# AssemblyAI-Community/MinImagen

Hardware: NVIDIA H100
Metric: denoising steps/sec (SR256 U-Net, batch 32 per GPU per step) (higher is better)
Workload: dtype f16 tensor-core operands, f32 accumulate / residual stream

## Files before the change

minimagen_b200/csrc/conv_tc.cu:

```cuda
#include "conv_tc.cuh"

#include <cuda_runtime.h>
#include <mutex>
#include <stdio.h>

#include "kernels.cuh"
#include "launch.cuh"
#include "ptx.cuh"
#include "sat_half.cuh"
#include "wgmma.cuh"

namespace mi {

namespace {

constexpr int kNumThreads = 384;
constexpr uint32_t kABytes = kConvBlockM * kConvBlockK * 2;
constexpr uint32_t kRingBudget = 192 * 1024;
constexpr uint32_t kAuxBytes = 512;
constexpr uint32_t kSmemMax = 227 * 1024;
constexpr int kProducerRegs = 40;
constexpr int kConsumerRegs = 232;
static_assert(128 * kProducerRegs + 256 * kConsumerRegs <= 65536, "register file overcommitted");
constexpr int kTurnBar = 2;
constexpr int kStatBar = 4;
constexpr uint32_t stat_scratch_bytes(int block_n) { return 2 * 4 * (block_n / 16 > 0 ? block_n / 16 : 1) * 2 * 8; }

template <int BLOCK_N>
struct Cfg {
    static constexpr uint32_t kBBytes = BLOCK_N * kConvBlockK * 2;
    static constexpr uint32_t kStageBytes = kABytes + kBBytes;
    static constexpr int kStages = (kRingBudget / kStageBytes) > 8 ? 8 : (kRingBudget / kStageBytes);
    static constexpr uint32_t kSmemBytes = kStages * kStageBytes + 1024  + kAuxBytes;
};

__device__ __forceinline__ float silu(float v) { return __fdividef(v, 1.0f + __expf(-v)); }

template <int BLOCK_N, bool GN>
__global__ void __launch_bounds__(kNumThreads, 1)
conv_wg_kernel(const __grid_constant__ CUtensorMap tmA, const __grid_constant__ CUtensorMap tmA2,
               const __grid_constant__ CUtensorMap tmB, const __grid_constant__ CUtensorMap tmX,
               const __grid_constant__ CUtensorMap tmX2, const __grid_constant__ ConvTcArgs args,
               const __grid_constant__ GnPrologueArgs gn) {
    using C = Cfg<BLOCK_N>;
    constexpr int STAGES = C::kStages;
    static_assert(2 * STAGES * 8 <= 256, "barrier block overlaps the GroupNorm scratch");
    constexpr bool PP = !GN && BLOCK_N <= 128;
    constexpr int HALVES = PP ? 2 : 1;

    extern __shared__ uint8_t smem_raw[];
    uint8_t* smem = reinterpret_cast<uint8_t*>((reinterpret_cast<uintptr_t>(smem_raw) + 1023) & ~uintptr_t(1023));
    uint64_t* bars = reinterpret_cast<uint64_t*>(smem + STAGES * C::kStageBytes);
    uint64_t* full_bar = bars;
    uint64_t* empty_bar = bars + STAGES;

    const int warp = threadIdx.x >> 5;
    const int lane = threadIdx.x & 31;
    const int wg = threadIdx.x >> 7;
    int* err = args.err_flag;

    if (threadIdx.x == 0) {
        ptx::prefetch_tensormap(&tmB);
        if (!GN) {
            ptx::prefetch_tensormap(&tmA);
            ptx::prefetch_tensormap(&tmA2);
        }
        for (int i = 0; i < STAGES; ++i) {
            ptx::mbar_init(&full_bar[i], GN ? 5 : 1);
            ptx::mbar_init(&empty_bar[i], PP ? 1 : 2);
        }
        ptx::fence_barrier_init();
    }
    __syncthreads();
    pdl_wait();

    const int num_tap_kb = args.num_taps * args.chunks_per_tap;
    const int num_kb = num_tap_kb + args.x_chunks;
    const int tiles_m = args.tiles_w * args.tiles_h * args.tiles_b;
    const int total_tiles = tiles_m * args.tiles_n;
    const int BW = 1 << args.bw_log2, BH = 1 << args.bh_log2;
    const int BB = kConvBlockM >> (args.bw_log2 + args.bh_log2);

    if (wg == 0) {
        if constexpr (!GN) {
            ptx::setmaxnreg_dec<kProducerRegs>();
            if (warp == 0) {
                int stage = 0;
                uint32_t phase = 0;
                for (int tile = blockIdx.x; tile < total_tiles; tile += gridDim.x) {
                    const int nt = tile % args.tiles_n;
                    const int mt = tile / args.tiles_n;
                    const int w0 = (mt % args.tiles_w) * BW;
                    const int h0 = ((mt / args.tiles_w) % args.tiles_h) * BH;
                    const int b0 = (mt / (args.tiles_w * args.tiles_h)) * BB;
                    const int n0 = nt * BLOCK_N;
                    for (int kb = 0; kb < num_kb; ++kb) {
                        ptx::mbar_wait(&empty_bar[stage], phase ^ 1, err, 100 + stage);
                        if (ptx::elect_one()) {
                            uint8_t* sa = smem + stage * C::kStageBytes;
                            uint8_t* sb = sa + kABytes;
                            ptx::mbar_arrive_expect_tx(&full_bar[stage], C::kStageBytes);
                            if (kb < num_tap_kb) {
                                const int t = kb / args.chunks_per_tap, j = kb - t * args.chunks_per_tap;
                                const int cw = w0 * args.in_stride + args.dw[t], ch = h0 * args.in_stride + args.dh[t];
                                if (j < args.a_split)
                                    ptx::tma_load_5d(&tmA, &full_bar[stage], sa, args.a_chan_off + j * kConvBlockK, cw, ch,
                                                     args.ph[t], b0);
                                else
                                    ptx::tma_load_5d(&tmA2, &full_bar[stage], sa,
                                                     args.a_chan_off2 + (j - args.a_split) * kConvBlockK, cw, ch, args.ph[t], b0);
                            } else {
                                const int jx = kb - num_tap_kb;
                                if (jx < args.x_split)
                                    ptx::tma_load_5d(&tmX, &full_bar[stage], sa, args.x_chan_off + jx * kConvBlockK, w0, h0, 0, b0);
                                else
                                    ptx::tma_load_5d(&tmX2, &full_bar[stage], sa,
                                                     args.x_chan_off2 + (jx - args.x_split) * kConvBlockK, w0, h0, 0, b0);
                            }
                            ptx::tma_load_2d(&tmB, &full_bar[stage], sb, kb * kConvBlockK, n0);
                        }
                        if (++stage == STAGES) { stage = 0; phase ^= 1; }
                    }
                }
                pdl_trigger();
            }
        } else {
            float* s_mean = reinterpret_cast<float*>(reinterpret_cast<uint8_t*>(bars) + 256);
            float* s_rstd = s_mean + 32;
            float* sA = reinterpret_cast<float*>(reinterpret_cast<uint8_t*>(bars) + kAuxBytes);
            const int tt = threadIdx.x;
            const int lq = tt & 7;
            const int prow = tt >> 3;
            const int C0 = gn.C0, C1 = gn.C1, Ctot = C0 + C1, Cg = Ctot / gn.groups;
            const int H = args.H, W = args.W;
            float* sB = sA + Ctot;
            int stage = 0;
            uint32_t phase = 0;
            int cur_b = -1;
            for (int tile = blockIdx.x; tile < total_tiles; tile += gridDim.x) {
                const int nt = tile % args.tiles_n;
                const int mt = tile / args.tiles_n;
                const int w0 = (mt % args.tiles_w) * BW;
                const int h0 = ((mt / args.tiles_w) % args.tiles_h) * BH;
                const int b = mt / (args.tiles_w * args.tiles_h);
                const int n0 = nt * BLOCK_N;
                if (b != cur_b) {
                    ptx::bar_sync(1, 128);
                    if (tt < gn.groups) {
                        const int g = tt;
                        double su = 0.0, sq = 0.0;
                        const int lo = g * Cg, hi = lo + Cg;
                        const int lo0 = min(lo, C0), hi0 = min(hi, C0);
                        for (int e = lo0 / 16; e < hi0 / 16; ++e) {
                            su += gn.stats0[((long long)b * (C0 / 16) + e) * 2];
                            sq += gn.stats0[((long long)b * (C0 / 16) + e) * 2 + 1];
                        }
                        const int lo1 = max(lo, C0) - C0, hi1 = max(hi, C0) - C0;
                        for (int e = lo1 / 16; e < hi1 / 16; ++e) {
                            su += (double)gn.scale1 * gn.stats1[((long long)b * (C1 / 16) + e) * 2];
                            sq += (double)gn.scale1 * (double)gn.scale1 * gn.stats1[((long long)b * (C1 / 16) + e) * 2 + 1];
                        }
                        const double n = (double)Cg * H * W;
                        const double mean = su / n;
                        double var = sq / n - mean * mean;
                        if (var < 0) var = 0;
                        s_mean[g] = (float)mean;
                        s_rstd[g] = (float)(1.0 / sqrt(var + (double)gn.eps));
                    }
                    ptx::bar_sync(1, 128);
                    for (int cc = tt; cc < Ctot; cc += 128) {
                        const int g = cc / Cg;
                        float a = s_rstd[g] * gn.gamma[cc];
                        float bb = gn.beta[cc] - s_mean[g] * a;
                        if (gn.scale_shift) {
                            const float sc = gn.scale_shift[(long long)b * gn.ss_ld + cc] + 1.0f;
                            const float shv = gn.scale_shift[(long long)b * gn.ss_ld + Ctot + cc];
                            a *= sc;
                            bb = bb * sc + shv;
                        }
                        if (cc >= C0) a *= gn.scale1;
                        sA[cc] = a;
                        sB[cc] = bb;
                    }
                    cur_b = b;
                    ptx::bar_sync(1, 128);
                }
                const long long img = (long long)b * H * W;
                for (int kb = 0; kb < num_kb; ++kb) {
                    const int t = kb / args.chunks_per_tap, j = kb - t * args.chunks_per_tap;
                    const int dh = args.dh[t], dw = args.dw[t];
                    const float* cA = sA + j * kConvBlockK + lq * 8;
                    const float* cB = sB + j * kConvBlockK + lq * 8;
                    const float4 a0 = *reinterpret_cast<const float4*>(cA), a1 = *reinterpret_cast<const float4*>(cA + 4);
                    const float4 b0 = *reinterpret_cast<const float4*>(cB), b1 = *reinterpret_cast<const float4*>(cB + 4);
                    const bool first = j < args.a_split;
                    const int Cs = first ? C0 : C1;
                    const float* src = (first ? gn.src0 + (long long)j * kConvBlockK
                                              : gn.src1 + (long long)(j - args.a_split) * kConvBlockK) + img * Cs + lq * 8;

                    ptx::mbar_wait(&empty_bar[stage], phase ^ 1, err, 600 + stage);
                    uint8_t* sa = smem + stage * C::kStageBytes;
                    if (warp == 0 && ptx::elect_one()) {
                        ptx::mbar_arrive_expect_tx(&full_bar[stage], C::kBBytes);
                        ptx::tma_load_2d(&tmB, &full_bar[stage], sa + kABytes, kb * kConvBlockK, n0);
                    }
                    float4 x0[8], x1[8];
                    bool ok[8];
#pragma unroll
                    for (int i = 0; i < 8; ++i) {
                        const int m = i * 16 + prow;
                        const int gw = w0 + (m & (BW - 1)) + dw;
                        const int gh = h0 + ((m >> args.bw_log2) & (BH - 1)) + dh;
                        ok[i] = gh >= 0 && gh < H && gw >= 0 && gw < W;
                        if (ok[i]) {
                            const float4* s4 = reinterpret_cast<const float4*>(src + ((long long)gh * W + gw) * Cs);
                            x0[i] = __ldg(s4);
                            x1[i] = __ldg(s4 + 1);
                        }
                    }
#pragma unroll
                    for (int i = 0; i < 8; ++i) {
                        const int m = i * 16 + prow;
                        uint4 o = make_uint4(0u, 0u, 0u, 0u);
                        if (ok[i]) {
                            const __half2 h0_ = sat_half2(silu(fmaf(x0[i].x, a0.x, b0.x)), silu(fmaf(x0[i].y, a0.y, b0.y)));
                            const __half2 h1_ = sat_half2(silu(fmaf(x0[i].z, a0.z, b0.z)), silu(fmaf(x0[i].w, a0.w, b0.w)));
                            const __half2 h2_ = sat_half2(silu(fmaf(x1[i].x, a1.x, b1.x)), silu(fmaf(x1[i].y, a1.y, b1.y)));
                            const __half2 h3_ = sat_half2(silu(fmaf(x1[i].z, a1.z, b1.z)), silu(fmaf(x1[i].w, a1.w, b1.w)));
                            o.x = *reinterpret_cast<const uint32_t*>(&h0_); o.y = *reinterpret_cast<const uint32_t*>(&h1_);
                            o.z = *reinterpret_cast<const uint32_t*>(&h2_); o.w = *reinterpret_cast<const uint32_t*>(&h3_);
                        }
                        *reinterpret_cast<uint4*>(sa + m * 128 + ((lq ^ (m & 7)) << 4)) = o;
                    }
                    ptx::fence_proxy_async_smem();
                    __syncwarp();
                    if (lane == 0) ptx::mbar_arrive(&full_bar[stage]);
                    if (++stage == STAGES) { stage = 0; phase ^= 1; }
                }
            }
            pdl_trigger();
        }
    } else {
        if constexpr (!GN) ptx::setmaxnreg_inc<kConsumerRegs>();
        const int cw = wg - 1;
        const int wq = warp & 3;
        const int cq = 2 * (lane & 3);
        float acc[HALVES][BLOCK_N / 2];
        int stage = 0;
        uint32_t phase = 0;
        auto skip = [&](int n) {
            stage += n % STAGES;
            phase ^= (uint32_t)(n / STAGES) & 1u;
            if (stage >= STAGES) { stage -= STAGES; phase ^= 1; }
        };
        if (PP) skip(cw * num_kb);
        int bw_r[2 * HALVES], bh_r[2 * HALVES], bb_r[2 * HALVES], bb_warp[HALVES];
#pragma unroll
        for (int h = 0; h < HALVES; ++h) {
            const int m_warp = (PP ? h : cw) * 64 + wq * 16;
            bb_warp[h] = m_warp >> (args.bw_log2 + args.bh_log2);
#pragma unroll
            for (int r = 0; r < 2; ++r) {
                const int m = m_warp + (lane >> 2) + 8 * r;
                bw_r[2 * h + r] = m & (BW - 1);
                bh_r[2 * h + r] = (m >> args.bw_log2) & (BH - 1);
                bb_r[2 * h + r] = m >> (args.bw_log2 + args.bh_log2);
            }
        }
        constexpr int NQ = BLOCK_N / 16 > 0 ? BLOCK_N / 16 : 1;
        const bool tile_stats = PP && args.stats != nullptr && BB == 1;
        double* st_red = reinterpret_cast<double*>(reinterpret_cast<uint8_t*>(bars) + kAuxBytes);
        const bool vec = args.out_sc == 1 && ((reinterpret_cast<uintptr_t>(args.out_f32) & 7) == 0) &&
                         ((reinterpret_cast<uintptr_t>(args.residual) & 7) == 0) &&
                         ((reinterpret_cast<uintptr_t>(args.out_f16) & 3) == 0);

        for (int tile = blockIdx.x + (PP ? cw : 0) * gridDim.x; tile < total_tiles; tile += (PP ? 2 : 1) * gridDim.x) {
            const int nt = tile % args.tiles_n;
            const int mt = tile / args.tiles_n;
            const int n0 = nt * BLOCK_N;
            if (PP && tile != (int)blockIdx.x) ptx::bar_sync(kTurnBar + cw, 256);
            int prev = -1;
            for (int kb = 0; kb < num_kb; ++kb) {
                ptx::mbar_wait(&full_bar[stage], phase, err, 300 + stage);
                const uint32_t sa = ptx::smem_u32(smem + stage * C::kStageBytes);
                const uint64_t db = ptx::make_sw128_desc(sa + kABytes);
                ptx::wg_fence();
#pragma unroll
                for (int k = 0; k < kConvBlockK / 16; ++k)
#pragma unroll
                    for (int h = 0; h < HALVES; ++h) {
                        const uint64_t da = ptx::make_sw128_desc(sa + (PP ? h : cw) * (64 * 128));
                        ptx::Wgmma<BLOCK_N, 0>::run(acc[h], da + 2 * k, db + 2 * k, (kb | k) != 0);
                    }
                ptx::wg_commit();
                ptx::wg_wait<1>();
                if (prev >= 0 && (threadIdx.x & 127) == 0) ptx::mbar_arrive(&empty_bar[prev]);
                prev = stage;
                if (++stage == STAGES) { stage = 0; phase ^= 1; }
            }
            if (PP && tile + (int)gridDim.x < total_tiles) ptx::bar_arrive(kTurnBar + (cw ^ 1), 256);
            if (PP) skip(num_kb);
            ptx::wg_wait<0>();
#pragma unroll
            for (int h = 0; h < HALVES; ++h) ptx::wg_fence_regs(acc[h]);
            if (prev >= 0 && (threadIdx.x & 127) == 0) ptx::mbar_arrive(&empty_bar[prev]);

            const int tw0 = (mt % args.tiles_w) * BW;
            const int th0 = ((mt / args.tiles_w) % args.tiles_h) * BH;
            const int tb0 = (mt / (args.tiles_w * args.tiles_h)) * BB;
            const bool fast = vec && n0 + BLOCK_N <= args.n_valid;
#pragma unroll
            for (int hf = 0; hf < HALVES; ++hf) {
                bool valid[2];
                long long pix[2];
#pragma unroll
                for (int r = 0; r < 2; ++r) {
                    const int w = tw0 + bw_r[2 * hf + r], h = th0 + bh_r[2 * hf + r], b = tb0 + bb_r[2 * hf + r];
                    valid[r] = (b < args.B) && (h < args.H) && (w < args.W);
                    pix[r] = (long long)b * args.out_sb + (long long)h * args.out_sh + (long long)w * args.out_sw;
                }
                const float* a = acc[hf];
                float st_s[BLOCK_N / 16 > 0 ? BLOCK_N / 16 : 1], st_q[BLOCK_N / 16 > 0 ? BLOCK_N / 16 : 1];
#pragma unroll
                for (int q = 0; q < BLOCK_N / 16; ++q) { st_s[q] = 0.f; st_q[q] = 0.f; }
#pragma unroll
                for (int j = 0; j < BLOCK_N / 8; ++j) {
                    const int n = n0 + 8 * j + cq;
                    if (fast) {
                        float2 bv = make_float2(0.f, 0.f);
                        if (args.bias) bv = __ldg(reinterpret_cast<const float2*>(args.bias + n));
#pragma unroll
                        for (int r = 0; r < 2; ++r) {
                            if (!valid[r]) continue;
                            const long long o = pix[r] + n;
                            float2 f = make_float2(a[4 * j + 2 * r] + bv.x, a[4 * j + 2 * r + 1] + bv.y);
                            if (args.residual) {
                                const float2 rv = *reinterpret_cast<const float2*>(args.residual + o);
                                f.x += rv.x; f.y += rv.y;
                            }
                            st_s[j >> 1] += f.x + f.y;
                            st_q[j >> 1] += f.x * f.x + f.y * f.y;
                            if (args.out_f32) *reinterpret_cast<float2*>(args.out_f32 + o) = f;
                            if (args.out_f16) *reinterpret_cast<__half2*>(args.out_f16 + o) = sat_half2(f.x, f.y);
                        }
                    } else {
#pragma unroll
                        for (int r = 0; r < 2; ++r) {
#pragma unroll
                            for (int e = 0; e < 2; ++e) {
                                if (!valid[r] || n + e >= args.n_valid) continue;
                                float f = a[4 * j + 2 * r + e] + (args.bias ? __ldg(args.bias + n + e) : 0.f);
                                const long long o = pix[r] + (long long)(n + e) * args.out_sc;
                                if (args.residual && args.out_sc == 1) f += args.residual[o];
                                st_s[j >> 1] += f;
                                st_q[j >> 1] += f * f;
                                if (args.out_f32) args.out_f32[o] = f;
                                if (args.out_f16) args.out_f16[o] = sat_half(f);
                            }
                        }
                    }
                }
                if (args.stats) {
                    const int b_img = tb0 + bb_warp[hf];
                    const bool any = __any_sync(0xffffffffu, valid[0] || valid[1]);
#pragma unroll
                    for (int q = 0; q < BLOCK_N / 16; ++q) {
#pragma unroll
                        for (int o = 1; o <= 16; o <<= 1) {
                            st_s[q] += __shfl_xor_sync(0xffffffffu, st_s[q], o);
                            st_q[q] += __shfl_xor_sync(0xffffffffu, st_q[q], o);
                        }
                        if (lane == 0 && tile_stats) {
                            double* r = st_red + ((cw * 4 + wq) * NQ + q) * 2;
                            r[0] = (hf == 0 ? 0.0 : r[0]) + (double)st_s[q];
                            r[1] = (hf == 0 ? 0.0 : r[1]) + (double)st_q[q];
                        } else if (lane == 0 && any) {
                            double* dst = args.stats + ((long long)b_img * args.stats_blocks + (n0 >> 4) + q) * 2;
                            atomicAdd(dst, (double)st_s[q]);
                            atomicAdd(dst + 1, (double)st_q[q]);
                        }
                    }
                }
            }
            if (tile_stats) {
                ptx::bar_sync(kStatBar + cw, 128);
                if (wq == 0 && lane < NQ) {
                    const double* r = st_red + (cw * 4 * NQ + lane) * 2;
                    double s = r[0], sq = r[1];
#pragma unroll
                    for (int w = 1; w < 4; ++w) { s += r[w * NQ * 2]; sq += r[w * NQ * 2 + 1]; }
                    double* dst = args.stats + ((long long)tb0 * args.stats_blocks + (n0 >> 4) + lane) * 2;
                    atomicAdd(dst, s);
                    atomicAdd(dst + 1, sq);
                }
                ptx::bar_sync(kStatBar + cw, 128);
            }
        }
    }
}


typedef CUresult (*PFN_encodeTiled)(CUtensorMap*, CUtensorMapDataType, cuuint32_t, void*, const cuuint64_t*,
                                    const cuuint64_t*, const cuuint32_t*, const cuuint32_t*, CUtensorMapInterleave,
                                    CUtensorMapSwizzle, CUtensorMapL2promotion, CUtensorMapFloatOOBfill);

PFN_encodeTiled get_encode() {
    static PFN_encodeTiled fn = nullptr;
    static std::once_flag once;
    std::call_once(once, [] {
        void* p = nullptr;
        cudaDriverEntryPointQueryResult q;
        if (cudaGetDriverEntryPoint("cuTensorMapEncodeTiled", &p, cudaEnableDefault, &q) == cudaSuccess &&
            q == cudaDriverEntryPointSuccess)
            fn = reinterpret_cast<PFN_encodeTiled>(p);
    });
    return fn;
}

int ilog2_exact(int v) {
    int l = 0;
    while ((1 << l) < v) ++l;
    return ((1 << l) == v) ? l : -1;
}

int num_sms_of_current_device() {
    int dev = 0;
    cudaGetDevice(&dev);
    static int cache[64] = {0};
    if (dev < 64 && cache[dev] != 0) return cache[dev];
    int n = 0;
    cudaDeviceGetAttribute(&n, cudaDevAttrMultiProcessorCount, dev);
    if (dev < 64) cache[dev] = n;
    return n;
}

void tile_geometry(int H, int W, int B, ConvTcArgs& a) {
    int BW = W >= 128 ? 128 : W;
    int BH = 128 / BW;
    if (BH > H) BH = H;
    const int BB = 128 / (BW * BH);
    a.bw_log2 = ilog2_exact(BW);
    a.bh_log2 = ilog2_exact(BH);
    a.tiles_w = (W + BW - 1) / BW;
    a.tiles_h = H / BH;
    a.tiles_b = (B + BB - 1) / BB;
    a.B = B; a.H = H; a.W = W;
}

int pick_block_n(int Cout, int tiles_m, int hint, int num_sms) {
    const int cands[5] = {256, 128, 64, 32, 16};
    if (hint < 0) hint = -hint;
    if (hint > 0 && Cout % hint == 0)
        for (int i = 0; i < 5; ++i)
            if (cands[i] == hint) return hint;
    int block_n = 16;
    for (int i = 0; i < 5; ++i) {
        if (Cout % cands[i] != 0) continue;
        block_n = cands[i];
        if (tiles_m * (Cout / cands[i]) >= num_sms || cands[i] <= 64) break;
    }
    return block_n;
}

CUresult encode_act(PFN_encodeTiled enc, CUtensorMap* m, const void* ptr, cuuint64_t channels, cuuint64_t ld, int W, int H,
                    int phases, int B, int in_stride, const ConvTcArgs& a) {
    const cuuint64_t IS = in_stride;
    const int BW = 1 << a.bw_log2, BH = 1 << a.bh_log2, BB = kConvBlockM >> (a.bw_log2 + a.bh_log2);
    cuuint64_t gdim[5] = {channels, (cuuint64_t)W * IS, (cuuint64_t)H * IS, (cuuint64_t)phases, (cuuint64_t)B};
    cuuint64_t gstr[4] = {ld * 2, (cuuint64_t)W * IS * ld * 2, (cuuint64_t)H * IS * W * IS * ld * 2,
                          (cuuint64_t)phases * H * IS * W * IS * ld * 2};
    cuuint32_t box[5] = {kConvBlockK, (cuuint32_t)(BW * IS), (cuuint32_t)(BH * IS), 1, (cuuint32_t)BB};
    cuuint32_t estr[5] = {1, (cuuint32_t)IS, (cuuint32_t)IS, 1, 1};
    return enc(m, CU_TENSOR_MAP_DATA_TYPE_FLOAT16, 5, const_cast<void*>(ptr), gdim, gstr, box, estr,
               CU_TENSOR_MAP_INTERLEAVE_NONE, CU_TENSOR_MAP_SWIZZLE_128B, CU_TENSOR_MAP_L2_PROMOTION_L2_256B,
               CU_TENSOR_MAP_FLOAT_OOB_FILL_NONE);
}

CUresult encode_weights(PFN_encodeTiled enc, CUtensorMap* m, const void* ptr, cuuint64_t K, int Cout, int block_n) {
    cuuint64_t gdim[2] = {K, (cuuint64_t)Cout};
    cuuint64_t gstr[1] = {K * 2};
    cuuint32_t box[2] = {kConvBlockK, (cuuint32_t)block_n};
    cuuint32_t estr[2] = {1, 1};
    return enc(m, CU_TENSOR_MAP_DATA_TYPE_FLOAT16, 2, const_cast<void*>(ptr), gdim, gstr, box, estr,
               CU_TENSOR_MAP_INTERLEAVE_NONE, CU_TENSOR_MAP_SWIZZLE_128B, CU_TENSOR_MAP_L2_PROMOTION_L2_256B,
               CU_TENSOR_MAP_FLOAT_OOB_FILL_NONE);
}

template <int BLOCK_N, bool GN>
int launch(const CUtensorMap& tmA, const CUtensorMap& tmA2, const CUtensorMap& tmB, const CUtensorMap& tmX,
           const CUtensorMap& tmX2, const ConvTcArgs& args, const GnPrologueArgs& gn, uint32_t extra_smem,
           cudaStream_t stream) {
    using C = Cfg<BLOCK_N>;
    static bool attr_set = false;
    if (!attr_set) {
        if (cudaFuncSetAttribute(conv_wg_kernel<BLOCK_N, GN>, cudaFuncAttributeMaxDynamicSharedMemorySize, kSmemMax) !=
            cudaSuccess)
            return -10;
        attr_set = true;
    }
    const int total_tiles = args.tiles_w * args.tiles_h * args.tiles_b * args.tiles_n;
    const int num_sms = num_sms_of_current_device();
    const int grid = total_tiles < num_sms ? total_tiles : num_sms;
    const uint32_t smem = C::kSmemBytes + (!GN && BLOCK_N <= 128 ? stat_scratch_bytes(BLOCK_N) : 0u) + extra_smem;
    launch_k(conv_wg_kernel<BLOCK_N, GN>, grid, kNumThreads, smem, stream, tmA, tmA2, tmB, tmX, tmX2, args, gn);
    return cudaGetLastError() == cudaSuccess ? 0 : -11;
}

}

PFN_tmaEncodeTiled get_tma_encode() { return get_encode(); }

const char* conv_tc_strerror(int code) {
    switch (code) {
        case 0: return "ok";
        case -1: return "conv_tc: C_in (per tap) must be a positive multiple of 64";
        case -2: return "conv_tc: C_out must be a multiple of 16";
        case -3: return "conv_tc: W must be a power of two >= 8 or a multiple of 128; H*W tiling unsupported";
        case -4: return "conv_tc: too many taps (max 16)";
        case -5: return "conv_tc: cuTensorMapEncodeTiled unavailable";
        case -6: return "conv_tc: tensor map encode failed (activations)";
        case -7: return "conv_tc: tensor map encode failed (weights)";
        case -8: return "conv_tc: pointer/stride alignment (16 B) violated";
        case -9: return "conv_tc: the folded 1x1 operand needs a stride-1 conv over one phase";
        case -10: return "conv_tc: cudaFuncSetAttribute(max dynamic smem) failed";
        case -11: return "conv_tc: kernel launch failed";
        default: return "conv_tc: unknown error";
    }
}

bool conv_tc_supported(int H, int W, int Cin, int Cout) {
    if (Cin <= 0 || Cin % kConvBlockK != 0 || Cout <= 0 || Cout % 16 != 0) return false;
    if (W >= 128) return true;
    if (ilog2_exact(W) < 3) return false;
    const int bh = 128 / W;
    if (H >= bh) return H % bh == 0;
    return ilog2_exact(H) >= 0;
}

int conv_tc_launch(const ConvTcProblem& p, cudaStream_t stream) {
    if (p.Cin <= 0 || p.Cin % kConvBlockK != 0) return -1;
    if (p.Cout % 16 != 0) return -2;
    if (p.num_taps < 1 || p.num_taps > kConvMaxTaps) return -4;
    if (!conv_tc_supported(p.H, p.W, p.Cin, p.Cout)) return -3;
    if ((reinterpret_cast<uintptr_t>(p.act) & 15) || (reinterpret_cast<uintptr_t>(p.wpacked) & 15) ||
        (p.lda % 8) != 0)
        return -8;
    PFN_encodeTiled enc = get_encode();
    if (!enc) return -5;

    ConvTcArgs a{};
    a.num_taps = p.num_taps;
    a.chunks_per_tap = p.Cin / kConvBlockK;
    tile_geometry(p.H, p.W, p.B, a);
    a.a_chan_off = p.a_chan_off;
    a.in_stride = p.in_stride == 2 ? 2 : 1;
    a.out_sb = p.out_sb; a.out_sh = p.out_sh; a.out_sw = p.out_sw;
    a.out_sc = p.out_sc > 0 ? p.out_sc : 1;
    a.n_valid = p.n_valid > 0 ? p.n_valid : p.Cout;
    a.out_f32 = p.out_f32; a.out_f16 = p.out_f16; a.bias = p.bias; a.residual = p.residual;
    a.err_flag = p.err_flag;
    a.stats = p.stats; a.stats_blocks = p.Cout / 16;
    for (int t = 0; t < p.num_taps; ++t) { a.dh[t] = p.dh[t]; a.dw[t] = p.dw[t]; a.ph[t] = p.ph[t]; }

    const int tiles_m = a.tiles_w * a.tiles_h * a.tiles_b;
    const int block_n = pick_block_n(p.Cout, tiles_m, p.block_n_hint, num_sms_of_current_device());
    a.tiles_n = p.Cout / block_n;

    CUtensorMap tmA, tmA2, tmB, tmX, tmX2;
    a.a_split = (p.act2 ? p.Cin1 : p.Cin) / kConvBlockK;
    a.a_chan_off2 = p.a_chan_off2;
    if (encode_act(enc, &tmA, p.act, p.a_channels, p.lda, p.W, p.H, p.phases, p.B, a.in_stride, a) != CUDA_SUCCESS) return -6;
    tmA2 = tmA;
    if (p.act2) {
        if (p.Cin1 <= 0 || p.Cin1 % kConvBlockK || p.Cin1 >= p.Cin || (p.lda2 % 8) || (reinterpret_cast<uintptr_t>(p.act2) & 15) ||
            a.in_stride != 1)
            return -8;
        if (encode_act(enc, &tmA2, p.act2, p.lda2, p.lda2, p.W, p.H, p.phases, p.B, 1, a) != CUDA_SUCCESS) return -6;
    }
    tmX = tmA; tmX2 = tmA;
    if (p.x_act) {
        if (p.phases != 1 || a.in_stride != 1) return -9;
        if (p.Cx <= 0 || p.Cx % kConvBlockK || (p.x_lda % 8) || (reinterpret_cast<uintptr_t>(p.x_act) & 15)) return -8;
        if (p.x_act2 && (p.Cx1 <= 0 || p.Cx1 % kConvBlockK || p.Cx1 >= p.Cx || (p.x_lda2 % 8) ||
                         (reinterpret_cast<uintptr_t>(p.x_act2) & 15)))
            return -8;
        a.x_chunks = p.Cx / kConvBlockK;
        a.x_split = (p.x_act2 ? p.Cx1 : p.Cx) / kConvBlockK;
        a.x_chan_off = p.x_chan_off; a.x_chan_off2 = p.x_chan_off2;
        if (encode_act(enc, &tmX, p.x_act, p.x_lda, p.x_lda, p.W, p.H, 1, p.B, 1, a) != CUDA_SUCCESS) return -6;
        tmX2 = tmX;
        if (p.x_act2 && encode_act(enc, &tmX2, p.x_act2, p.x_lda2, p.x_lda2, p.W, p.H, 1, p.B, 1, a) != CUDA_SUCCESS) return -6;
    }
    const cuuint64_t K = (cuuint64_t)p.num_taps * p.Cin + (p.x_act ? (cuuint64_t)p.Cx : 0);
    if (encode_weights(enc, &tmB, p.wpacked, K, p.Cout, block_n) != CUDA_SUCCESS) return -7;

    const GnPrologueArgs gn{};
    switch (block_n) {
        case 256: return launch<256, false>(tmA, tmA2, tmB, tmX, tmX2, a, gn, 0, stream);
        case 128: return launch<128, false>(tmA, tmA2, tmB, tmX, tmX2, a, gn, 0, stream);
        case 64: return launch<64, false>(tmA, tmA2, tmB, tmX, tmX2, a, gn, 0, stream);
        case 32: return launch<32, false>(tmA, tmA2, tmB, tmX, tmX2, a, gn, 0, stream);
        default: return launch<16, false>(tmA, tmA2, tmB, tmX, tmX2, a, gn, 0, stream);
    }
}


bool conv_gn_supported(int H, int W, int C0, int C1, int Cout, int groups) {
    const int C = C0 + C1;
    if (H <= 0 || W <= 0 || H % 32 || W % 8 || C0 <= 0 || C0 % 64 || C1 < 0 || C1 % 64 || Cout <= 0 || Cout % 128) return false;
    if (!conv_tc_supported(H, W, C, Cout) || H * W < kConvBlockM) return false;
    if (groups < 1 || groups > 32 || C % groups) return false;
    if (Cfg<128>::kSmemBytes + 8u * (uint32_t)C > kSmemMax) return false;
    return (C / groups) % 16 == 0;
}

int conv_gn_launch(const ConvGnProblem& p, cudaStream_t stream) {
    if (!conv_gn_supported(p.H, p.W, p.C0, p.C1, p.Cout, p.groups)) return -3;
    if (p.C1 && (!p.src1 || !p.stats1)) return -8;
    if (!p.src0 || !p.stats0 || !p.gamma || !p.beta) return -8;
    if ((reinterpret_cast<uintptr_t>(p.src0) & 15) || (reinterpret_cast<uintptr_t>(p.src1) & 15) ||
        (reinterpret_cast<uintptr_t>(p.wpacked) & 15))
        return -8;
    PFN_encodeTiled enc = get_encode();
    if (!enc) return -5;
    const int C = p.C0 + p.C1;

    ConvTcArgs a{};
    a.num_taps = 9;
    for (int t = 0; t < 9; ++t) { a.dh[t] = (int8_t)(t / 3 - 1); a.dw[t] = (int8_t)(t % 3 - 1); a.ph[t] = 0; }
    a.chunks_per_tap = C / kConvBlockK;
    a.a_split = p.C0 / kConvBlockK;
    a.in_stride = 1;
    tile_geometry(p.H, p.W, p.B, a);
    a.out_sb = (long long)p.H * p.W * p.Cout; a.out_sh = (long long)p.W * p.Cout; a.out_sw = p.Cout; a.out_sc = 1;
    a.n_valid = p.Cout;
    a.out_f32 = p.out_f32; a.out_f16 = p.out_f16; a.bias = p.bias; a.residual = p.residual; a.err_flag = p.err_flag;
    a.stats = p.out_stats; a.stats_blocks = p.Cout / 16;
    a.tiles_n = p.Cout / 128;

    GnPrologueArgs g{};
    g.src0 = p.src0; g.src1 = p.src1;
    g.C0 = p.C0; g.C1 = p.C1; g.groups = p.groups; g.scale1 = p.scale1; g.eps = p.eps;
    g.stats0 = p.stats0; g.stats1 = p.stats1; g.gamma = p.gamma; g.beta = p.beta;
    g.scale_shift = p.scale_shift; g.ss_ld = p.ss_ld;

    CUtensorMap tmB;
    if (encode_weights(enc, &tmB, p.wpacked, (cuuint64_t)9 * C, p.Cout, 128) != CUDA_SUCCESS) return -7;
    return launch<128, true>(tmB, tmB, tmB, tmB, tmB, a, g, 8u * (uint32_t)C, stream);
}

}
```

minimagen_b200/csrc/conv_tc.cuh:

```cuda
#pragma once
#include <cuda_fp16.h>
#include <cuda_runtime.h>
#include <stdint.h>

namespace mi {

constexpr int kConvBlockM = 128;
constexpr int kConvBlockK = 64;
constexpr int kConvMaxTaps = 16;

struct ConvTcArgs {
    int num_taps, chunks_per_tap;
    int bw_log2, bh_log2;
    int tiles_w, tiles_h, tiles_b, tiles_n;
    int B, H, W;
    int a_chan_off;
    int in_stride;
    int a_split, a_chan_off2;
    int x_chunks, x_split;
    int x_chan_off, x_chan_off2;
    long long out_sb, out_sh, out_sw;
    long long out_sc;
    int n_valid;
    float* out_f32;
    __half* out_f16;
    const float* bias;
    const float* residual;
    int* err_flag;
    double* stats;
    int stats_blocks;
    int8_t dh[kConvMaxTaps], dw[kConvMaxTaps], ph[kConvMaxTaps];
};

struct ConvTcProblem {
    const void* act;
    int B, H, W;
    int phases;
    int in_stride;
    int lda;
    int a_channels;
    int a_chan_off;
    int Cin;
    const void* act2;
    int lda2, a_chan_off2, Cin1;
    const void* wpacked;
    int Cout;
    const void* x_act; int x_lda, x_chan_off, Cx;
    const void* x_act2; int x_lda2, x_chan_off2, Cx1;
    int num_taps;
    int8_t dh[kConvMaxTaps], dw[kConvMaxTaps], ph[kConvMaxTaps];
    float* out_f32; __half* out_f16; const float* bias; const float* residual;
    long long out_sb, out_sh, out_sw;
    long long out_sc;
    int n_valid;
    int block_n_hint;
    double* stats;
    int* err_flag;
};

struct GnPrologueArgs {
    const float* src0;
    const float* src1;
    int C0, C1, groups;
    float scale1, eps;
    const double* stats0;
    const double* stats1;
    const float* gamma;
    const float* beta;
    const float* scale_shift;
    int ss_ld;
};

struct ConvGnProblem {
    const float* src0; int C0;
    const float* src1; int C1;
    float scale1;
    int B, H, W, groups;
    const double* stats0; const double* stats1;
    const float* gamma; const float* beta; const float* scale_shift; int ss_ld; float eps;
    const void* wpacked; int Cout;
    const float* bias; const float* residual;
    float* out_f32; __half* out_f16; double* out_stats;
    int* err_flag;
};

bool conv_gn_supported(int H, int W, int C0, int C1, int Cout, int groups);
int conv_gn_launch(const ConvGnProblem& p, cudaStream_t stream);

bool conv_tc_supported(int H, int W, int Cin, int Cout);
int conv_tc_launch(const ConvTcProblem& p, cudaStream_t stream);
const char* conv_tc_strerror(int code);

}
```

Baseline: 15.66.

## Load one tall activation box per tap row and reuse it across vertical taps

Splits the shared-memory ring into separate A and B rings with their own barriers. For dense 3x3 convolutions it loads one taller A box covering BH+rows-1 image rows per horizontal tap group, and the consumer offsets the descriptor by r*BW rows to serve each vertical tap from that box. This is meant to cut activation TMA traffic roughly threefold. In exchange it uses narrower 32-wide tiles, fewer A stages, more complex barrier bookkeeping, and it changes tiles_h to ceiling division.

```diff
diff --git a/minimagen_b200/csrc/conv_tc.cu b/minimagen_b200/csrc/conv_tc.cu
--- a/minimagen_b200/csrc/conv_tc.cu
+++ b/minimagen_b200/csrc/conv_tc.cu
@@ -16,7 +16,9 @@
 
 constexpr int kNumThreads = 384;
 constexpr uint32_t kABytes = kConvBlockM * kConvBlockK * 2;
+constexpr uint32_t kRowBoxMax = 24 * 1024;
 constexpr uint32_t kRingBudget = 192 * 1024;
+constexpr int kMaxSlots = 8;
 constexpr uint32_t kAuxBytes = 512;
 constexpr uint32_t kSmemMax = 227 * 1024;
 constexpr int kProducerRegs = 40;
@@ -29,10 +31,17 @@
 template <int BLOCK_N>
 struct Cfg {
     static constexpr uint32_t kBBytes = BLOCK_N * kConvBlockK * 2;
-    static constexpr uint32_t kStageBytes = kABytes + kBBytes;
-    static constexpr int kStages = (kRingBudget / kStageBytes) > 8 ? 8 : (kRingBudget / kStageBytes);
-    static constexpr uint32_t kSmemBytes = kStages * kStageBytes + 1024  + kAuxBytes;
+    static constexpr int kBStages =
+        (kRingBudget / (kABytes + kBBytes)) > kMaxSlots ? kMaxSlots : (kRingBudget / (kABytes + kBBytes));
+    static_assert(kRingBudget - (kBStages - 1) * kBBytes >= 3 * kRowBoxMax, "three row boxes must fit the A ring");
+    static constexpr uint32_t kSmemBytes = kRingBudget + 1024  + kAuxBytes;
 };
+
+template <int BLOCK_N>
+__device__ __forceinline__ int b_slots(uint32_t a_slot) {
+    using C = Cfg<BLOCK_N>;
+    return (kRingBudget - C::kBStages * C::kBBytes) / a_slot >= 3 ? C::kBStages : C::kBStages - 1;
+}
 
 __device__ __forceinline__ float silu(float v) { return __fdividef(v, 1.0f + __expf(-v)); }
 
@@ -43,16 +52,17 @@
                const __grid_constant__ CUtensorMap tmX2, const __grid_constant__ ConvTcArgs args,
                const __grid_constant__ GnPrologueArgs gn) {
     using C = Cfg<BLOCK_N>;
-    constexpr int STAGES = C::kStages;
-    static_assert(2 * STAGES * 8 <= 256, "barrier block overlaps the GroupNorm scratch");
+    static_assert(4 * kMaxSlots * 8 <= 256, "barrier block overlaps the GroupNorm scratch");
     constexpr bool PP = !GN && BLOCK_N <= 128;
     constexpr int HALVES = PP ? 2 : 1;
 
     extern __shared__ uint8_t smem_raw[];
     uint8_t* smem = reinterpret_cast<uint8_t*>((reinterpret_cast<uintptr_t>(smem_raw) + 1023) & ~uintptr_t(1023));
-    uint64_t* bars = reinterpret_cast<uint64_t*>(smem + STAGES * C::kStageBytes);
-    uint64_t* full_bar = bars;
-    uint64_t* empty_bar = bars + STAGES;
+    uint64_t* bars = reinterpret_cast<uint64_t*>(smem + kRingBudget);
+    uint64_t* full_a = bars;
+    uint64_t* empty_a = bars + kMaxSlots;
+    uint64_t* full_b = bars + 2 * kMaxSlots;
+    uint64_t* empty_b = bars + 3 * kMaxSlots;
 
     const int warp = threadIdx.x >> 5;
     const int lane = threadIdx.x & 31;
@@ -65,28 +75,41 @@
             ptx::prefetch_tensormap(&tmA);
             ptx::prefetch_tensormap(&tmA2);
         }
-        for (int i = 0; i < STAGES; ++i) {
-            ptx::mbar_init(&full_bar[i], GN ? 5 : 1);
-            ptx::mbar_init(&empty_bar[i], PP ? 1 : 2);
+        for (int i = 0; i < kMaxSlots; ++i) {
+            ptx::mbar_init(&full_a[i], GN ? 4 : 1);
+            ptx::mbar_init(&empty_a[i], PP ? 1 : 2);
+            ptx::mbar_init(&full_b[i], 1);
+            ptx::mbar_init(&empty_b[i], PP ? 1 : 2);
         }
         ptx::fence_barrier_init();
     }
     __syncthreads();
     pdl_wait();
 
-    const int num_tap_kb = args.num_taps * args.chunks_per_tap;
+    const int cpt = args.chunks_per_tap;
+    const int num_tap_kb = args.num_taps * cpt;
     const int num_kb = num_tap_kb + args.x_chunks;
     const int tiles_m = args.tiles_w * args.tiles_h * args.tiles_b;
     const int total_tiles = tiles_m * args.tiles_n;
     const int BW = 1 << args.bw_log2, BH = 1 << args.bh_log2;
     const int BB = kConvBlockM >> (args.bw_log2 + args.bh_log2);
+    const int rows = args.a_rows;
+    const int groups = args.num_taps / rows;
+    const int num_tap_a = groups * cpt;
+    const int num_a = num_tap_a + args.x_chunks;
+    const uint32_t a_slot = kABytes + (uint32_t)(rows - 1) * BW * 128;
+    const int NB = b_slots<BLOCK_N>(a_slot);
+    const uint32_t a_ring_bytes = kRingBudget - NB * C::kBBytes;
+    const int NA = (int)(a_ring_bytes / a_slot) < kMaxSlots ? (int)(a_ring_bytes / a_slot) : kMaxSlots;
+    uint8_t* b_ring = smem;
+    uint8_t* a_ring = smem + NB * C::kBBytes;
 
     if (wg == 0) {
         if constexpr (!GN) {
             ptx::setmaxnreg_dec<kProducerRegs>();
             if (warp == 0) {
-                int stage = 0;
-                uint32_t phase = 0;
+                int sa = 0, sb = 0;
+                uint32_t pa = 0, pb = 0;
                 for (int tile = blockIdx.x; tile < total_tiles; tile += gridDim.x) {
                     const int nt = tile % args.tiles_n;
                     const int mt = tile / args.tiles_n;
@@ -94,32 +117,42 @@
                     const int h0 = ((mt / args.tiles_w) % args.tiles_h) * BH;
                     const int b0 = (mt / (args.tiles_w * args.tiles_h)) * BB;
                     const int n0 = nt * BLOCK_N;
-                    for (int kb = 0; kb < num_kb; ++kb) {
-                        ptx::mbar_wait(&empty_bar[stage], phase ^ 1, err, 100 + stage);
+                    for (int i = 0; i < num_a; ++i) {
+                        const bool tap = i < num_tap_a;
+                        const int g = i / cpt, j = i - g * cpt;
+                        ptx::mbar_wait(&empty_a[sa], pa ^ 1, err, 100 + sa);
                         if (ptx::elect_one()) {
-                            uint8_t* sa = smem + stage * C::kStageBytes;
-                            uint8_t* sb = sa + kABytes;
-                            ptx::mbar_arrive_expect_tx(&full_bar[stage], C::kStageBytes);
-                            if (kb < num_tap_kb) {
-                                const int t = kb / args.chunks_per_tap, j = kb - t * args.chunks_per_tap;
-                                const int cw = w0 * args.in_stride + args.dw[t], ch = h0 * args.in_stride + args.dh[t];
+                            uint8_t* dst = a_ring + sa * a_slot;
+                            if (tap) {
+                                ptx::mbar_arrive_expect_tx(&full_a[sa], a_slot);
+                                const int cw = w0 * args.in_stride + args.dw[g], ch = h0 * args.in_stride + args.dh[g];
                                 if (j < args.a_split)
-                                    ptx::tma_load_5d(&tmA, &full_bar[stage], sa, args.a_chan_off + j * kConvBlockK, cw, ch,
-                                                     args.ph[t], b0);
+                                    ptx::tma_load_5d(&tmA, &full_a[sa], dst, args.a_chan_off + j * kConvBlockK, cw, ch,
+                                                     args.ph[g], b0);
                                 else
-                                    ptx::tma_load_5d(&tmA2, &full_bar[stage], sa,
-                                                     args.a_chan_off2 + (j - args.a_split) * kConvBlockK, cw, ch, args.ph[t], b0);
+                                    ptx::tma_load_5d(&tmA2, &full_a[sa], dst,
+                                                     args.a_chan_off2 + (j - args.a_split) * kConvBlockK, cw, ch, args.ph[g], b0);
                             } else {
-                                const int jx = kb - num_tap_kb;
+                                ptx::mbar_arrive_expect_tx(&full_a[sa], kABytes);
+                                const int jx = i - num_tap_a;
                                 if (jx < args.x_split)
-                                    ptx::tma_load_5d(&tmX, &full_bar[stage], sa, args.x_chan_off + jx * kConvBlockK, w0, h0, 0, b0);
+                                    ptx::tma_load_5d(&tmX, &full_a[sa], dst, args.x_chan_off + jx * kConvBlockK, w0, h0, 0, b0);
                                 else
-                                    ptx::tma_load_5d(&tmX2, &full_bar[stage], sa,
+                                    ptx::tma_load_5d(&tmX2, &full_a[sa], dst,
                                                      args.x_chan_off2 + (jx - args.x_split) * kConvBlockK, w0, h0, 0, b0);
                             }
-                            ptx::tma_load_2d(&tmB, &full_bar[stage], sb, kb * kConvBlockK, n0);
-                        }
-                        if (++stage == STAGES) { stage = 0; phase ^= 1; }
+                        }
+                        if (++sa == NA) { sa = 0; pa ^= 1; }
+                        const int nk = tap ? rows : 1;
+                        for (int r = 0; r < nk; ++r) {
+                            ptx::mbar_wait(&empty_b[sb], pb ^ 1, err, 200 + sb);
+                            if (ptx::elect_one()) {
+                                const int kcol = tap ? (r * groups + g) * cpt + j : num_tap_kb + (i - num_tap_a);
+                                ptx::mbar_arrive_expect_tx(&full_b[sb], C::kBBytes);
+                                ptx::tma_load_2d(&tmB, &full_b[sb], b_ring + sb * C::kBBytes, kcol * kConvBlockK, n0);
+                            }
+                            if (++sb == NB) { sb = 0; pb ^= 1; }
+                        }
                     }
                 }
                 pdl_trigger();
@@ -134,8 +167,8 @@
             const int C0 = gn.C0, C1 = gn.C1, Ctot = C0 + C1, Cg = Ctot / gn.groups;
             const int H = args.H, W = args.W;
             float* sB = sA + Ctot;
-            int stage = 0;
-            uint32_t phase = 0;
+            int sa = 0, sb = 0;
+            uint32_t pa = 0, pb = 0;
             int cur_b = -1;
             for (int tile = blockIdx.x; tile < total_tiles; tile += gridDim.x) {
                 const int nt = tile % args.tiles_n;
@@ -198,11 +231,12 @@
                     const float* src = (first ? gn.src0 + (long long)j * kConvBlockK
                                               : gn.src1 + (long long)(j - args.a_split) * kConvBlockK) + img * Cs + lq * 8;
 
-                    ptx::mbar_wait(&empty_bar[stage], phase ^ 1, err, 600 + stage);
-                    uint8_t* sa = smem + stage * C::kStageBytes;
+                    ptx::mbar_wait(&empty_a[sa], pa ^ 1, err, 600 + sa);
+                    ptx::mbar_wait(&empty_b[sb], pb ^ 1, err, 700 + sb);
+                    uint8_t* dst = a_ring + sa * a_slot;
                     if (warp == 0 && ptx::elect_one()) {
-                        ptx::mbar_arrive_expect_tx(&full_bar[stage], C::kBBytes);
-                        ptx::tma_load_2d(&tmB, &full_bar[stage], sa + kABytes, kb * kConvBlockK, n0);
+                        ptx::mbar_arrive_expect_tx(&full_b[sb], C::kBBytes);
+                        ptx::tma_load_2d(&tmB, &full_b[sb], b_ring + sb * C::kBBytes, kb * kConvBlockK, n0);
                     }
                     float4 x0[8], x1[8];
                     bool ok[8];
@@ -230,12 +264,13 @@
                             o.x = *reinterpret_cast<const uint32_t*>(&h0_); o.y = *reinterpret_cast<const uint32_t*>(&h1_);
                             o.z = *reinterpret_cast<const uint32_t*>(&h2_); o.w = *reinterpret_cast<const uint32_t*>(&h3_);
                         }
-                        *reinterpret_cast<uint4*>(sa + m * 128 + ((lq ^ (m & 7)) << 4)) = o;
+                        *reinterpret_cast<uint4*>(dst + m * 128 + ((lq ^ (m & 7)) << 4)) = o;
                     }
                     ptx::fence_proxy_async_smem();
                     __syncwarp();
-                    if (lane == 0) ptx::mbar_arrive(&full_bar[stage]);
-                    if (++stage == STAGES) { stage = 0; phase ^= 1; }
+                    if (lane == 0) ptx::mbar_arrive(&full_a[sa]);
+                    if (++sa == NA) { sa = 0; pa ^= 1; }
+                    if (++sb == NB) { sb = 0; pb ^= 1; }
                 }
             }
             pdl_trigger();
@@ -246,14 +281,14 @@
         const int wq = warp & 3;
         const int cq = 2 * (lane & 3);
         float acc[HALVES][BLOCK_N / 2];
-        int stage = 0;
-        uint32_t phase = 0;
-        auto skip = [&](int n) {
-            stage += n % STAGES;
-            phase ^= (uint32_t)(n / STAGES) & 1u;
-            if (stage >= STAGES) { stage -= STAGES; phase ^= 1; }
+        int sa = 0, sb = 0;
+        uint32_t pa = 0, pb = 0;
+        auto skip = [](int& s, uint32_t& p, int n, int slots) {
+            s += n % slots;
+            p ^= (uint32_t)(n / slots) & 1u;
+            if (s >= slots) { s -= slots; p ^= 1; }
         };
-        if (PP) skip(cw * num_kb);
+        if (PP && cw) { skip(sa, pa, num_a, NA); skip(sb, pb, num_kb, NB); }
         int bw_r[2 * HALVES], bh_r[2 * HALVES], bb_r[2 * HALVES], bb_warp[HALVES];
 #pragma unroll
         for (int h = 0; h < HALVES; ++h) {
@@ -279,31 +314,44 @@
             const int mt = tile / args.tiles_n;
             const int n0 = nt * BLOCK_N;
             if (PP && tile != (int)blockIdx.x) ptx::bar_sync(kTurnBar + cw, 256);
-            int prev = -1;
-            for (int kb = 0; kb < num_kb; ++kb) {
-                ptx::mbar_wait(&full_bar[stage], phase, err, 300 + stage);
-                const uint32_t sa = ptx::smem_u32(smem + stage * C::kStageBytes);
-                const uint64_t db = ptx::make_sw128_desc(sa + kABytes);
-                ptx::wg_fence();
-#pragma unroll
-                for (int k = 0; k < kConvBlockK / 16; ++k)
-#pragma unroll
-                    for (int h = 0; h < HALVES; ++h) {
-                        const uint64_t da = ptx::make_sw128_desc(sa + (PP ? h : cw) * (64 * 128));
-                        ptx::Wgmma<BLOCK_N, 0>::run(acc[h], da + 2 * k, db + 2 * k, (kb | k) != 0);
-                    }
-                ptx::wg_commit();
-                ptx::wg_wait<1>();
-                if (prev >= 0 && (threadIdx.x & 127) == 0) ptx::mbar_arrive(&empty_bar[prev]);
-                prev = stage;
-                if (++stage == STAGES) { stage = 0; phase ^= 1; }
+            int prev_a = -1, prev_b = -1;
+            int kb = 0;
+            for (int i = 0; i < num_a; ++i) {
+                const int nk = i < num_tap_a ? rows : 1;
+                ptx::mbar_wait(&full_a[sa], pa, err, 300 + sa);
+                const uint32_t a_base = ptx::smem_u32(a_ring + sa * a_slot);
+                for (int r = 0; r < nk; ++r, ++kb) {
+                    ptx::mbar_wait(&full_b[sb], pb, err, 400 + sb);
+                    const uint64_t db = ptx::make_sw128_desc(ptx::smem_u32(b_ring + sb * C::kBBytes));
+                    ptx::wg_fence();
+#pragma unroll
+                    for (int k = 0; k < kConvBlockK / 16; ++k)
+#pragma unroll
+                        for (int h = 0; h < HALVES; ++h) {
+                            const uint64_t da = ptx::make_sw128_desc(a_base + (r * BW + (PP ? h : cw) * 64) * 128);
+                            ptx::Wgmma<BLOCK_N, 0>::run(acc[h], da + 2 * k, db + 2 * k, (kb | k) != 0);
+                        }
+                    ptx::wg_commit();
+                    ptx::wg_wait<1>();
+                    if ((threadIdx.x & 127) == 0) {
+                        if (prev_b >= 0) ptx::mbar_arrive(&empty_b[prev_b]);
+                        if (prev_a >= 0) ptx::mbar_arrive(&empty_a[prev_a]);
+                    }
+                    prev_b = sb;
+                    prev_a = r == nk - 1 ? sa : -1;
+                    if (++sb == NB) { sb = 0; pb ^= 1; }
+                }
+                if (++sa == NA) { sa = 0; pa ^= 1; }
             }
             if (PP && tile + (int)gridDim.x < total_tiles) ptx::bar_arrive(kTurnBar + (cw ^ 1), 256);
-            if (PP) skip(num_kb);
+            if (PP) { skip(sa, pa, num_a, NA); skip(sb, pb, num_kb, NB); }
             ptx::wg_wait<0>();
 #pragma unroll
             for (int h = 0; h < HALVES; ++h) ptx::wg_fence_regs(acc[h]);
-            if (prev >= 0 && (threadIdx.x & 127) == 0) ptx::mbar_arrive(&empty_bar[prev]);
+            if ((threadIdx.x & 127) == 0) {
+                if (prev_b >= 0) ptx::mbar_arrive(&empty_b[prev_b]);
+                if (prev_a >= 0) ptx::mbar_arrive(&empty_a[prev_a]);
+            }
 
             const int tw0 = (mt % args.tiles_w) * BW;
             const int th0 = ((mt / args.tiles_w) % args.tiles_h) * BH;
@@ -434,15 +482,34 @@
     return n;
 }
 
-void tile_geometry(int H, int W, int B, ConvTcArgs& a) {
-    int BW = W >= 128 ? 128 : W;
-    int BH = 128 / BW;
-    if (BH > H) BH = H;
+int grid_rows(const ConvTcProblem& p) {
+    if (p.phases != 1 || p.in_stride == 2) return 1;
+    int kw = 1;
+    while (kw < p.num_taps && p.dh[kw] == p.dh[0]) ++kw;
+    if (p.num_taps % kw) return 1;
+    for (int t = 0; t < p.num_taps; ++t)
+        if (p.dh[t] != p.dh[0] + t / kw || p.dw[t] != p.dw[0] + t % kw || p.ph[t] != 0) return 1;
+    return p.num_taps / kw;
+}
+
+void tile_geometry(int H, int W, int B, int rows, ConvTcArgs& a) {
+    int BW, BH;
+    if (rows > 1) {
+        BW = W >= 32 ? 32 : W;
+        BH = 128 / BW;
+        if (H < BH || (uint32_t)(BH + rows - 1) * BW * 128 > kRowBoxMax) rows = 1;
+    }
+    if (rows == 1) {
+        BW = W >= 128 ? 128 : W;
+        BH = 128 / BW;
+        if (BH > H) BH = H;
+    }
     const int BB = 128 / (BW * BH);
+    a.a_rows = rows;
     a.bw_log2 = ilog2_exact(BW);
     a.bh_log2 = ilog2_exact(BH);
     a.tiles_w = (W + BW - 1) / BW;
-    a.tiles_h = H / BH;
+    a.tiles_h = (H + BH - 1) / BH;
     a.tiles_b = (B + BB - 1) / BB;
     a.B = B; a.H = H; a.W = W;
 }
@@ -463,13 +530,13 @@
 }
 
 CUresult encode_act(PFN_encodeTiled enc, CUtensorMap* m, const void* ptr, cuuint64_t channels, cuuint64_t ld, int W, int H,
-                    int phases, int B, int in_stride, const ConvTcArgs& a) {
+                    int phases, int B, int in_stride, int rows, const ConvTcArgs& a) {
     const cuuint64_t IS = in_stride;
     const int BW = 1 << a.bw_log2, BH = 1 << a.bh_log2, BB = kConvBlockM >> (a.bw_log2 + a.bh_log2);
     cuuint64_t gdim[5] = {channels, (cuuint64_t)W * IS, (cuuint64_t)H * IS, (cuuint64_t)phases, (cuuint64_t)B};
     cuuint64_t gstr[4] = {ld * 2, (cuuint64_t)W * IS * ld * 2, (cuuint64_t)H * IS * W * IS * ld * 2,
                           (cuuint64_t)phases * H * IS * W * IS * ld * 2};
-    cuuint32_t box[5] = {kConvBlockK, (cuuint32_t)(BW * IS), (cuuint32_t)(BH * IS), 1, (cuuint32_t)BB};
+    cuuint32_t box[5] = {kConvBlockK, (cuuint32_t)(BW * IS), (cuuint32_t)((BH + rows - 1) * IS), 1, (cuuint32_t)BB};
     cuuint32_t estr[5] = {1, (cuuint32_t)IS, (cuuint32_t)IS, 1, 1};
     return enc(m, CU_TENSOR_MAP_DATA_TYPE_FLOAT16, 5, const_cast<void*>(ptr), gdim, gstr, box, estr,
                CU_TENSOR_MAP_INTERLEAVE_NONE, CU_TENSOR_MAP_SWIZZLE_128B, CU_TENSOR_MAP_L2_PROMOTION_L2_256B,
@@ -551,7 +618,7 @@
     ConvTcArgs a{};
     a.num_taps = p.num_taps;
     a.chunks_per_tap = p.Cin / kConvBlockK;
-    tile_geometry(p.H, p.W, p.B, a);
+    tile_geometry(p.H, p.W, p.B, grid_rows(p), a);
     a.a_chan_off = p.a_chan_off;
     a.in_stride = p.in_stride == 2 ? 2 : 1;
     a.out_sb = p.out_sb; a.out_sh = p.out_sh; a.out_sw = p.out_sw;
@@ -569,13 +636,14 @@
     CUtensorMap tmA, tmA2, tmB, tmX, tmX2;
     a.a_split = (p.act2 ? p.Cin1 : p.Cin) / kConvBlockK;
     a.a_chan_off2 = p.a_chan_off2;
-    if (encode_act(enc, &tmA, p.act, p.a_channels, p.lda, p.W, p.H, p.phases, p.B, a.in_stride, a) != CUDA_SUCCESS) return -6;
+    if (encode_act(enc, &tmA, p.act, p.a_channels, p.lda, p.W, p.H, p.phases, p.B, a.in_stride, a.a_rows, a) != CUDA_SUCCESS)
+        return -6;
     tmA2 = tmA;
     if (p.act2) {
         if (p.Cin1 <= 0 || p.Cin1 % kConvBlockK || p.Cin1 >= p.Cin || (p.lda2 % 8) || (reinterpret_cast<uintptr_t>(p.act2) & 15) ||
             a.in_stride != 1)
             return -8;
-        if (encode_act(enc, &tmA2, p.act2, p.lda2, p.lda2, p.W, p.H, p.phases, p.B, 1, a) != CUDA_SUCCESS) return -6;
+        if (encode_act(enc, &tmA2, p.act2, p.lda2, p.lda2, p.W, p.H, p.phases, p.B, 1, a.a_rows, a) != CUDA_SUCCESS) return -6;
     }
     tmX = tmA; tmX2 = tmA;
     if (p.x_act) {
@@ -587,9 +655,10 @@
         a.x_chunks = p.Cx / kConvBlockK;
         a.x_split = (p.x_act2 ? p.Cx1 : p.Cx) / kConvBlockK;
         a.x_chan_off = p.x_chan_off; a.x_chan_off2 = p.x_chan_off2;
-        if (encode_act(enc, &tmX, p.x_act, p.x_lda, p.x_lda, p.W, p.H, 1, p.B, 1, a) != CUDA_SUCCESS) return -6;
+        if (encode_act(enc, &tmX, p.x_act, p.x_lda, p.x_lda, p.W, p.H, 1, p.B, 1, 1, a) != CUDA_SUCCESS) return -6;
         tmX2 = tmX;
-        if (p.x_act2 && encode_act(enc, &tmX2, p.x_act2, p.x_lda2, p.x_lda2, p.W, p.H, 1, p.B, 1, a) != CUDA_SUCCESS) return -6;
+        if (p.x_act2 && encode_act(enc, &tmX2, p.x_act2, p.x_lda2, p.x_lda2, p.W, p.H, 1, p.B, 1, 1, a) != CUDA_SUCCESS)
+            return -6;
     }
     const cuuint64_t K = (cuuint64_t)p.num_taps * p.Cin + (p.x_act ? (cuuint64_t)p.Cx : 0);
     if (encode_weights(enc, &tmB, p.wpacked, K, p.Cout, block_n) != CUDA_SUCCESS) return -7;
@@ -631,7 +700,7 @@
     a.chunks_per_tap = C / kConvBlockK;
     a.a_split = p.C0 / kConvBlockK;
     a.in_stride = 1;
-    tile_geometry(p.H, p.W, p.B, a);
+    tile_geometry(p.H, p.W, p.B, 1, a);
     a.out_sb = (long long)p.H * p.W * p.Cout; a.out_sh = (long long)p.W * p.Cout; a.out_sw = p.Cout; a.out_sc = 1;
     a.n_valid = p.Cout;
     a.out_f32 = p.out_f32; a.out_f16 = p.out_f16; a.bias = p.bias; a.residual = p.residual; a.err_flag = p.err_flag;
diff --git a/minimagen_b200/csrc/conv_tc.cuh b/minimagen_b200/csrc/conv_tc.cuh
--- a/minimagen_b200/csrc/conv_tc.cuh
+++ b/minimagen_b200/csrc/conv_tc.cuh
@@ -11,6 +11,7 @@
 
 struct ConvTcArgs {
     int num_taps, chunks_per_tap;
+    int a_rows;
     int bw_log2, bh_log2;
     int tiles_w, tiles_h, tiles_b, tiles_n;
     int B, H, W;
```

New measurement: 16.00, median of 6. 1.02x the previous value.
